# shibatch/rectdetect

Measured on AMD Instinct MI355X. Metric: 1920x1080 frames/sec, higher is better.
Workload: dtype u8/i32/f32 (bit-exact integer + IEEE f32 stencil path)

## Files before the change

### rectdetect_amd/csrc/rd_front_helpers.h

```cpp
#pragma once
#include "rd_device.h"

namespace {
using namespace rd;

__device__ __forceinline__ float v5c(int i) {
  const float t[25] = {
    (float)-4.667, (float)-4.083, (float)0.000, (float)4.083, (float)4.667,
    (float)-10.024, (float)-0.963, (float)0.000, (float)0.963, (float)10.024,
    (float)-14.120, (float)3.622, (float)0.000, (float)-3.622, (float)14.120,
    (float)-10.024, (float)-0.963, (float)0.000, (float)0.963, (float)10.024,
    (float)-4.667, (float)-4.083, (float)0.000, (float)4.083, (float)4.667,
  };
  return t[i];
}

__device__ __forceinline__ float ep_strength(const float (&n)[3], const float (&s)[3], const float (&w)[3], const float (&e)[3],
                                             const float (&nw)[3], const float (&ne)[3], const float (&sw)[3], const float (&se)[3]) {
  float sum[3];
#pragma unroll
  for (int c = 0; c < 3; c++) {
    float t = n[c] + w[c] - s[c] - e[c];
    float acc = 0;
    acc += (nw[c] - se[c]) * t;
    t = n[c] - w[c] + e[c] - s[c];
    acc += (ne[c] - sw[c]) * t;
    sum[c] = fmaxf(0.0f, acc);
  }
  const float tot = sum[0] + sum[1] + sum[2];
  return tot > 0 ? sqrtf(tot) : 0.0f;
}

#define TT_PITCH 72
__device__ __forceinline__ float bicubic_lds(const float *t, float x, float y, int x0, int y0) {
  const int ix = (int)x, iy = (int)y;
  const float fx = x - ix, fy = y - iy;
  const float *q = t + (iy - 1 - (y0 - 3)) * TT_PITCH + (ix - 1 - (x0 - 3));
  float r[4];
#pragma unroll
  for (int k = 0; k < 4; k++) r[k] = cubic1(q[k * TT_PITCH], q[k * TT_PITCH + 1], q[k * TT_PITCH + 2], q[k * TT_PITCH + 3], fx);
  return cubic1(r[0], r[1], r[2], r[3], fy);
}

}
```

### rectdetect_amd/csrc/rd_k_nms.hip

```cpp
#include "rd_device.h"
#include "rd_kernels.h"
#include "rd_front_helpers.h"

namespace {

using namespace rd;

struct P3c { const float *p[3]; };
inline int cdiv(int a, int b) { return (a + b - 1) / b; }
const dim3 block2(64, 4);

#ifndef GN_ROWS
#define GN_ROWS 16
#endif
#define GN_LW 73
#define GN_LH (GN_ROWS + 9)
#define GN_SW 71
#define GN_SH (GN_ROWS + 7)
#ifndef GN_TY
#define GN_TY 4
#endif
#define GN_NT (64 * GN_TY)
#define GN_K (GN_ROWS / GN_TY)
struct GnTaps { uint32_t *plab1; float2 *vxy; float *strength; };

template <int TAPS>
__global__ __launch_bounds__(GN_NT) void k_grad_nms(float *__restrict__ out, P3c bl, int iw, int ih, size_t zs, GnTaps taps, int gdim) {
  const rd_tile rd_b = rd_block_tile(gdim);
  if (rd_b.x < 0) return;
  RD_ZSHIFTZ(rd_b.z, zs, out, bl.p[0], bl.p[1], bl.p[2], taps.plab1, taps.vxy, taps.strength);
  __shared__ float lab[4][GN_LH * GN_LW];
  __shared__ float str[GN_SH * TT_PITCH];
  __shared__ int nlst;
  static_assert(4 * GN_LH * GN_LW * 4 >= 64 * GN_ROWS * 20, "the list of maxima lives in the Lab tile's memory");
  const int x0 = rd_b.x * 64, y0 = rd_b.y * GN_ROWS;
  const int tx = threadIdx.x, ty = rd_ty(), tid = ty * 64 + tx;
  if (tid == 0) nlst = 0;
  {
    constexpr int NR = (GN_LH + GN_TY - 1) / GN_TY;
    const int mcol = mirror1(x0 - 4 + tx, iw);
    const int sc = tid < 9 * GN_LH ? tid : 0, scy = sc / 9, scx = 64 + sc - scy * 9;
    float vl[NR + 1], va[NR + 1], vb[NR + 1];
#pragma unroll
    for (int i = 0; i <= NR; i++) {
      const int cy = i < NR ? ty + GN_TY * i : scy, cx = i < NR ? tx : scx;
      const int fx = x0 - 4 + cx, fy = y0 - 4 + cy;
      const bool ok = cy < GN_LH && fx <= iw + 4 && fy <= ih + 4;
      const int a = ok ? mirror1(fy, ih) * iw + (i < NR ? mcol : mirror1(fx, iw)) : 0;
      vl[i] = bl.p[0][a]; va[i] = bl.p[1][a]; vb[i] = bl.p[2][a];
    }
#pragma unroll
    for (int i = 0; i <= NR; i++) {
      const int cy = i < NR ? ty + GN_TY * i : scy, cx = i < NR ? tx : scx;
      if (cy >= GN_LH || (i == NR && tid >= 9 * GN_LH)) continue;
      const int il = clampi(__float2int_rd(vl[i] * 4096), 0, 4095), ia = clampi(__float2int_rd(va[i] * 1024), 0, 1023), ib = clampi(__float2int_rd(vb[i] * 1024), 0, 1023);
      const int t = cy * GN_LW + cx;
      lab[0][t] = vl[i];
      lab[1][t] = (float)il * (1.0f / 4096) + 0.5f / 4096; lab[2][t] = (float)ia * (1.0f / 1024) + 0.5f / 1024; lab[3][t] = (float)ib * (1.0f / 1024) + 0.5f / 1024;
      if (TAPS) {
        const int fx = x0 - 4 + cx, fy = y0 - 4 + cy;
        if (cx >= 4 && cx < 68 && cy >= 4 && cy < 4 + GN_ROWS && fx < iw && fy < ih) taps.plab1[fy * iw + fx] = (uint32_t)il | ((uint32_t)ia << 12) | ((uint32_t)ib << 22);
      }
    }
  }
  __syncthreads();
  float2 dir[GN_K];
  {
    float w[GN_K + 4][5];
    const float *q = &lab[0][(ty * GN_K + 2) * GN_LW + tx + 2];
#pragma unroll
    for (int r = 0; r < GN_K + 4; r++)
#pragma unroll
      for (int c = 0; c < 5; c++) w[r][c] = q[r * GN_LW + c];
#pragma unroll
    for (int k = 0; k < GN_K; k++) {
      float vx = 0, vy = 0;
#pragma unroll
      for (int yy = -2; yy <= 2; yy++)
#pragma unroll
        for (int xx = -2; xx <= 2; xx++) {
          const float s = w[k + yy + 2][xx + 2];
          if (xx != 0) vx += v5c((xx + 2) + (yy + 2) * 5) * s;
          if (yy != 0) vy += v5c((yy + 2) + (xx + 2) * 5) * s;
        }
      float len = vx * vx + vy * vy;
      if ((double)len > 1e-10) { len = 1.0f / sqrtf(len); vx *= len; vy *= len; }
      else vx = vy = 0.70710678118f;
      dir[k] = make_float2(vx, vy);
      if (TAPS) { const int x = x0 + tx, y = y0 + ty * GN_K + k; if (x < iw && y < ih) taps.vxy[y * iw + x] = dir[k]; }
    }
  }
  const bool interior = x0 >= 3 && x0 + 67 < iw && y0 >= 3 && y0 + GN_ROWS + 3 < ih;
  auto strength_at = [&](int lx, int ly) {
    float n[3], s[3], w[3], e[3], nw[3], ne[3], sw[3], se[3];
    const int c = ly * GN_LW + lx;
#pragma unroll
    for (int k = 0; k < 3; k++) {
      const float *p = &lab[1 + k][c];
      nw[k] = p[-GN_LW - 1]; n[k] = p[-GN_LW]; ne[k] = p[-GN_LW + 1];
      w[k] = p[-1]; e[k] = p[1];
      sw[k] = p[GN_LW - 1]; s[k] = p[GN_LW]; se[k] = p[GN_LW + 1];
    }
    return ep_strength(n, s, w, e, nw, ne, sw, se);
  };
  if (interior) {
    constexpr int BAND = (GN_SH + GN_TY - 1) / GN_TY;
    const int r0 = ty * BAND, r1 = r0 + BAND < GN_SH ? r0 + BAND : GN_SH;
    {
      float u[BAND + 2][3][3];
#pragma unroll
      for (int r = 0; r < BAND + 2; r++) {
        const int ly = r0 + r < GN_LH - 1 ? r0 + r : GN_LH - 1;
#pragma unroll
        for (int c = 0; c < 3; c++)
#pragma unroll
          for (int k = 0; k < 3; k++) u[r][c][k] = lab[1 + k][ly * GN_LW + tx + c];
      }
#pragma unroll
      for (int r = 0; r < BAND; r++)
        if (r0 + r < r1) {
          const float v = ep_strength(u[r][1], u[r + 2][1], u[r + 1][0], u[r + 1][2], u[r][0], u[r][2], u[r + 2][0], u[r + 2][2]);
          str[(r0 + r) * TT_PITCH + tx] = v;
          if (TAPS) { const int sy = r0 + r; if (sy >= 3 && sy < 3 + GN_ROWS && tx >= 3) taps.strength[(y0 - 3 + sy) * iw + x0 - 3 + tx] = v; }
        }
    }
    for (int t = tid; t < 7 * GN_SH; t += GN_NT) {
      const int sy = t / 7, sx = 64 + t - sy * 7;
      const float v = strength_at(sx + 1, sy + 1);
      str[sy * TT_PITCH + sx] = v;
      if (TAPS) { if (sy >= 3 && sy < 3 + GN_ROWS && sx < 67) taps.strength[(y0 - 3 + sy) * iw + x0 - 3 + sx] = v; }
    }
  } else {
    for (int t = tid; t < GN_SW * GN_SH; t += GN_NT) {
      const int sy = t / GN_SW, sx = t - sy * GN_SW;
      const int fx = x0 - 3 + sx, fy = y0 - 3 + sy;
      if (fx > iw + 3 || fy > ih + 3) continue;
      const int mx = mirror1(fx, iw), my = mirror1(fy, ih);
      const float v = strength_at(mx - (x0 - 4), my - (y0 - 4));
      str[sy * TT_PITCH + sx] = v;
      if (TAPS) { if (sy >= 3 && sy < 3 + GN_ROWS && sx >= 3 && sx < 67 && fx < iw && fy < ih) taps.strength[fy * iw + fx] = v; }
    }
  }
  __syncthreads();
  float4 *lst = (float4 *)&lab[0][0];
  int *lpix = (int *)(lst + 64 * GN_ROWS);
  const int x = x0 + tx;
#pragma unroll
  for (int k = 0; k < GN_K; k++) {
    const int r = ty * GN_K + k;
    const int y = y0 + r;
    const bool inside = x < iw && y < ih;
    bool peak = false;
    float am1 = 0, ap1 = 0;
    const float2 v = dir[k];
    if (inside) {
      const float a0 = str[(r + 3) * TT_PITCH + tx + 3];
      am1 = bicubic_lds(str, x - 1 * v.x, y - 1 * v.y, x0, y0);
      ap1 = bicubic_lds(str, x + 1 * v.x, y + 1 * v.y, x0, y0);
      peak = am1 <= a0 && a0 >= ap1;
      if (!peak) out[y * iw + x] = 0.0f;
    }
    const unsigned long long m = __ballot(peak);
    if (m) {
      const int leader = __ffsll((long long)m) - 1;
      int b = 0;
      if (tx == leader) b = atomicAdd(&nlst, __popcll(m));
      b = __shfl(b, leader);
      if (peak) { const int i = b + __popcll(m & ((1ull << tx) - 1)); lst[i] = make_float4(am1, ap1, v.x, v.y); lpix[i] = r * 64 + tx; }
    }
  }
  __syncthreads();
  const int n = nlst;
  for (int i = tid; i < n; i += GN_NT) {
    const float4 e = lst[i];
    const int c = lpix[i], r = c >> 6, cx = c & 63;
    const int xx = x0 + cx, yy = y0 + r;
    const float a0 = str[(r + 3) * TT_PITCH + cx + 3];
    const float am2 = bicubic_lds(str, xx - 2 * e.z, yy - 2 * e.w, x0, y0);
    const float ap2 = bicubic_lds(str, xx + 2 * e.z, yy + 2 * e.w, x0, y0);
    out[yy * iw + xx] = am2 + e.x + a0 + e.y + ap2;
  }
}

}

namespace rdk {

int grad_nms_fits(int iw, int ih) {
  return iw >= 16 && ih >= 16 && (iw % 64 == 0 || iw % 64 >= 2) && (ih % GN_ROWS == 0 || ih % GN_ROWS >= 2);
}
void grad_nms(hipStream_t s, float *nms, float *const bl[3], int iw, int ih, int nz, size_t zs, uint32_t *tap_plab1, float *tap_vxy, float *tap_strength) {
  P3c b = { { bl[0], bl[1], bl[2] } };
  GnTaps t = { tap_plab1, (float2 *)tap_vxy, tap_strength };
  const dim3 grid(rd_tile_blocks(cdiv(iw, 64), cdiv(ih, GN_ROWS), nz));
  const int gdim = rd_gdim(cdiv(iw, 64), cdiv(ih, GN_ROWS), nz);
  if (tap_plab1) hipLaunchKernelGGL(k_grad_nms<1>, grid, dim3(64, GN_TY), 0, s, nms, b, iw, ih, zs, t, gdim);
  else hipLaunchKernelGGL(k_grad_nms<0>, grid, dim3(64, GN_TY), 0, s, nms, b, iw, ih, zs, t, gdim);
}
}
```

Measured before the change: 3164.

## Precompute per-row cubic coefficients in LDS for NMS bicubic sampling

Adds a pass that turns the strength tile into float4 horizontal cubic polynomial coefficients, stored in LDS that overlaps the Lab and strength tiles. Each bicubic sample then reads four float4 values and runs Horner steps in place of sixteen scalar loads plus the horizontal cubic math. The maxima list moves into the same shared memory with a fixed capacity, and peaks that overflow it are finished inline. This costs an extra LDS pass and barrier, and it may change float rounding versus the bit-exact reference cubic1 path.

```diff
diff --git a/rectdetect_amd/csrc/rd_front_helpers.h b/rectdetect_amd/csrc/rd_front_helpers.h
--- a/rectdetect_amd/csrc/rd_front_helpers.h
+++ b/rectdetect_amd/csrc/rd_front_helpers.h
@@ -42,4 +42,27 @@
   return cubic1(r[0], r[1], r[2], r[3], fy);
 }
 
+__device__ __forceinline__ float4 cubic_coef(float p0, float p1, float p2, float p3) {
+  const float v = p1 - p2, w = p3 - p0;
+  return make_float4(v * 3.0f + w, -4.0f * v + (p0 - p1 - w), p2 - p0, p1);
 }
+
+#define CF_PITCH 68
+__device__ __forceinline__ float bicubic(const float4 *t, float x, float y, int x0, int y0) {
+  const int ix = (int)x, iy = (int)y;
+  const float fx = x - ix, fy = y - iy;
+  const float4 *q = t + (iy - 1 - (y0 - 3)) * CF_PITCH + (ix - 1 - (x0 - 3));
+  float r[4];
+#pragma unroll
+  for (int k = 0; k < 4; k++) {
+    const float4 c = q[k * CF_PITCH];
+    float u = c.x;
+    u = u * fx + c.y;
+    u = u * fx + c.z;
+    u = u * fx * 0.5f + c.w;
+    r[k] = u;
+  }
+  return cubic1(r[0], r[1], r[2], r[3], fy);
+}
+
+}
diff --git a/rectdetect_amd/csrc/rd_k_nms.hip b/rectdetect_amd/csrc/rd_k_nms.hip
--- a/rectdetect_amd/csrc/rd_k_nms.hip
+++ b/rectdetect_amd/csrc/rd_k_nms.hip
@@ -22,6 +22,12 @@
 #endif
 #define GN_NT (64 * GN_TY)
 #define GN_K (GN_ROWS / GN_TY)
+#define GN_LAB (4 * GN_LH * GN_LW)
+#define GN_STR (GN_SH * TT_PITCH)
+#ifndef GN_LCAP
+#define GN_LCAP 540
+#endif
+static_assert(GN_SH * CF_PITCH * 16 + GN_LCAP * 20 <= (GN_LAB + GN_STR) * 4, "coefficient tile and list of maxima share the Lab and strength tiles' memory");
 struct GnTaps { uint32_t *plab1; float2 *vxy; float *strength; };
 
 template <int TAPS>
@@ -29,10 +35,13 @@
   const rd_tile rd_b = rd_block_tile(gdim);
   if (rd_b.x < 0) return;
   RD_ZSHIFTZ(rd_b.z, zs, out, bl.p[0], bl.p[1], bl.p[2], taps.plab1, taps.vxy, taps.strength);
-  __shared__ float lab[4][GN_LH * GN_LW];
-  __shared__ float str[GN_SH * TT_PITCH];
+  __shared__ __attribute__((aligned(16))) float smem[GN_LAB + GN_STR];
   __shared__ int nlst;
-  static_assert(4 * GN_LH * GN_LW * 4 >= 64 * GN_ROWS * 20, "the list of maxima lives in the Lab tile's memory");
+  float (*const lab)[GN_LH * GN_LW] = (float (*)[GN_LH * GN_LW])smem;
+  float *const str = smem + GN_LAB;
+  float4 *const cf = (float4 *)smem;
+  float4 *const lst = cf + GN_SH * CF_PITCH;
+  int *const lpix = (int *)(lst + GN_LCAP);
   const int x0 = rd_b.x * 64, y0 = rd_b.y * GN_ROWS;
   const int tx = threadIdx.x, ty = rd_ty(), tid = ty * 64 + tx;
   if (tid == 0) nlst = 0;
@@ -142,8 +151,20 @@
     }
   }
   __syncthreads();
-  float4 *lst = (float4 *)&lab[0][0];
-  int *lpix = (int *)(lst + 64 * GN_ROWS);
+  {
+    constexpr int NR = (GN_SH + GN_TY - 1) / GN_TY;
+#pragma unroll
+    for (int i = 0; i < NR; i++) {
+      const int r = ty + GN_TY * i;
+      if (r < GN_SH) { const float *p = &str[r * TT_PITCH + tx]; cf[r * CF_PITCH + tx] = cubic_coef(p[0], p[1], p[2], p[3]); }
+    }
+    if (tid < 4 * GN_SH) {
+      const int r = tid >> 2, c = 64 + (tid & 3);
+      const float *p = &str[r * TT_PITCH + c];
+      cf[r * CF_PITCH + c] = cubic_coef(p[0], p[1], p[2], p[3]);
+    }
+  }
+  __syncthreads();
   const int x = x0 + tx;
 #pragma unroll
   for (int k = 0; k < GN_K; k++) {
@@ -154,9 +175,9 @@
     float am1 = 0, ap1 = 0;
     const float2 v = dir[k];
     if (inside) {
-      const float a0 = str[(r + 3) * TT_PITCH + tx + 3];
-      am1 = bicubic_lds(str, x - 1 * v.x, y - 1 * v.y, x0, y0);
-      ap1 = bicubic_lds(str, x + 1 * v.x, y + 1 * v.y, x0, y0);
+      const float a0 = cf[(r + 3) * CF_PITCH + tx + 2].w;
+      am1 = bicubic(cf, x - 1 * v.x, y - 1 * v.y, x0, y0);
+      ap1 = bicubic(cf, x + 1 * v.x, y + 1 * v.y, x0, y0);
       peak = am1 <= a0 && a0 >= ap1;
       if (!peak) out[y * iw + x] = 0.0f;
     }
@@ -166,18 +187,27 @@
       int b = 0;
       if (tx == leader) b = atomicAdd(&nlst, __popcll(m));
       b = __shfl(b, leader);
-      if (peak) { const int i = b + __popcll(m & ((1ull << tx) - 1)); lst[i] = make_float4(am1, ap1, v.x, v.y); lpix[i] = r * 64 + tx; }
-    }
-  }
-  __syncthreads();
-  const int n = nlst;
+      if (peak) {
+        const int i = b + __popcll(m & ((1ull << tx) - 1));
+        if (i < GN_LCAP) { lst[i] = make_float4(am1, ap1, v.x, v.y); lpix[i] = r * 64 + tx; }
+        else {
+          const float a0 = cf[(r + 3) * CF_PITCH + tx + 2].w;
+          const float am2 = bicubic(cf, x - 2 * v.x, y - 2 * v.y, x0, y0);
+          const float ap2 = bicubic(cf, x + 2 * v.x, y + 2 * v.y, x0, y0);
+          out[y * iw + x] = am2 + am1 + a0 + ap1 + ap2;
+        }
+      }
+    }
+  }
+  __syncthreads();
+  const int n = nlst < GN_LCAP ? nlst : GN_LCAP;
   for (int i = tid; i < n; i += GN_NT) {
     const float4 e = lst[i];
     const int c = lpix[i], r = c >> 6, cx = c & 63;
     const int xx = x0 + cx, yy = y0 + r;
-    const float a0 = str[(r + 3) * TT_PITCH + cx + 3];
-    const float am2 = bicubic_lds(str, xx - 2 * e.z, yy - 2 * e.w, x0, y0);
-    const float ap2 = bicubic_lds(str, xx + 2 * e.z, yy + 2 * e.w, x0, y0);
+    const float a0 = cf[(r + 3) * CF_PITCH + cx + 2].w;
+    const float am2 = bicubic(cf, xx - 2 * e.z, yy - 2 * e.w, x0, y0);
+    const float ap2 = bicubic(cf, xx + 2 * e.z, yy + 2 * e.w, x0, y0);
     out[yy * iw + xx] = am2 + e.x + a0 + e.y + ap2;
   }
 }
```

New measurement: 3203 (median of 6 runs). 1.2% higher.
